# ARISE-Initiative/robosuite

Measured on AMD Instinct MI355X. Metric: env-steps/sec (whole node), Lift/Panda/OSC_POSE @4096 envs/GPU, higher is better.
Workload: dtype f32

## Files before the change

robosuite_amd/csrc/rsim_step.hip:

```cpp
#include <hip/hip_runtime.h>
#include <stdint.h>
#include <type_traits>

#include "../../include/rsim.h"
#include "rsim_internal.h"

#ifndef RSIM_CFG
#define RSIM_CFG 0
#endif
#if RSIM_CFG == 0
#define RSIM_DIMS 32, 16, 16, 24, 16, 16, 64, 192
#define RSIM_SYM(x) x##_cfg0
#define RSIM_DIMS_W 32, 16, 16, 24, 16, 32, 128, 192
#elif RSIM_CFG == 1
#define RSIM_DIMS 32, 16, 32, 24, 16, 32, 64, 192
#define RSIM_SYM(x) x##_cfg1
#define RSIM_DIMS_W 32, 16, 32, 24, 16, 32, 128, 192
#elif RSIM_CFG == 2
#define RSIM_DIMS 64, 16, 16, 32, 32, 32, 64, 320
#define RSIM_SYM(x) x##_cfg2
#define RSIM_DIMS_W 64, 16, 16, 32, 32, 32, 128, 320
#elif RSIM_CFG == 3
#define RSIM_DIMS 64, 32, 48, 64, 32, 32, 128, 640
#define RSIM_SYM(x) x##_cfg3
// ... 2975 lines not shown
    SYNC();
#pragma unroll
    for (int k = 0; k < NA; k++) lt6[k] = Lt[k * NA + (lane & (NA - 1))];
    {
      const float zl = rchol_solve_m<NA>(lr6, lt6, linv6, own6, lane < 6 ? vv[lane] : 0.f);
#pragma unroll
      for (int r = 0; r < 6; r++) z[r] = bcast(zl, r);
      if (!c.uncouple) {
        const float wl = rchol_solve_m<NA>(lr6, lt6, linv6, own6, lane < 3 ? F[lane] : (lane < 6 ? T[lane - 3] : 0.f));
#pragma unroll
        for (int r = 0; r < 6; r++) wrench[r] = bcast(wl, r);
      }
    }
    float tq = 0.f;
    if (lane < n) {
      tq = sm.qfrc_bias[di] + matmp;
#pragma unroll
      for (int r = 0; r < 6; r++) tq = fmaf(comp6(jc, r < 3 ? r + 3 : r - 3), wrench[r] - z[r], tq);
    }
    ctrl_write<ARM>(K, tq);
  }

  struct Row {
    float J[FAST ? NV16 : 1];
    float D, R, aref, fl, mu, fr_own, Dm;
    float fj[CD - 1];
    int row, type, head, kk, dim;
    bool valid, ell;
  };
  __device__ __forceinline__ float row_dot(const Row& rw, float x) const {
    if constexpr (FAST) return dot_rows<NV16>(rw.J, x);
    else return j_row_dot(rw.row * JS, x);
  }
  __device__ __forceinline__ float j_row_dot(int base, float x) const {
    if constexpr (!JG) return lds_row_dot(sm.J + base, x);
    else {
      float a[NV16];
#pragma unroll
      for (int u = 0; u < NV16; u++) a[u] = Jg[base + u];
      float acc = 0.f;
#pragma unroll
      for (int u = 0; u < NV16; u++) acc = fmaf(a[u], bcast(x, u), acc);
      return acc;
    }
  }
  __device__ __forceinline__ double row_res64(const Row& rw, float x, float xl) const {
    return j_row_res64(rw.row * JS, x, xl, rw.aref);
  }
  __device__ __forceinline__ double j_row_res64(int base, float x, float xl, float aref) const {
    if constexpr (!JG) return lds_row_res64(sm.J + base, x, xl, aref);
    else {
      float a[NV16];
#pragma unroll
      for (int u = 0; u < NV16; u++) a[u] = Jg[base + u];
      double acc = -(double)aref;
      float lo = 0.f;
#pragma unroll
      for (int u = 0; u < NV16; u++) { acc = fma((double)a[u], (double)bcast(x, u), acc); lo = fmaf(a[u], bcast(xl, u), lo); }
      return acc + (double)lo;
    }
  }
  __device__ __forceinline__ float lds_row_dot(const float* p, float x) const {
    float acc = 0.f;
    for (int k0 = 0; k0 < m.nv; k0 += 16) {
      float a[16];
#pragma unroll
      for (int u = 0; u < 16; u++) a[u] = p[k0 + u];
#pragma unroll
      for (int u = 0; u < 16; u++) acc = fmaf(a[u], bcast(x, k0 + u), acc);
    }
    return acc;
  }
  __device__ __forceinline__ double lds_row_res64(const float* p, float x, float xl, float aref) const {
    double acc = -(double)aref;
    float lo = 0.f;
    for (int k0 = 0; k0 < m.nv; k0 += 16) {
      float a[16];
#pragma unroll
      for (int u = 0; u < 16; u++) a[u] = p[k0 + u];
#pragma unroll
      for (int u = 0; u < 16; u++) { acc = fma((double)a[u], (double)bcast(x, k0 + u), acc); lo = fmaf(a[u], bcast(xl, k0 + u), lo); }
    }
    return acc + (double)lo;
  }
  __device__ __forceinline__ float mass_dot(const float (&Mr)[FAST ? NV16 : 1], float x) const {
    if constexpr (FAST) return dot_rows<NV16>(Mr, x);
    else {
      float acc;
      if constexpr (MG) {
        float a[NV16];
        const int base = (lane < m.nv ? lane : 0) * NVP;
#pragma unroll
        for (int u = 0; u < NV16; u++) a[u] = Mg[base + u];
        acc = 0.f;
#pragma unroll
        for (int u = 0; u < NV16; u++) acc = fmaf(a[u], bcast(x, u), acc);
      } else acc = lds_row_dot(sm.M + (lane < m.nv ? lane : 0) * NVP, x);
      return lane < m.nv ? acc : 0.f;
    }
  }
  __device__ __forceinline__ void gather(const Row (&rw)[NSLOT], const float (&x)[NSLOT], float (&out)[NSLOT][CD]) const {
    float u[NSLOT];
#pragma unroll
    for (int s = 0; s < NSLOT; s++) u[s] = x[s] * rw[s].fr_own;
#pragma unroll
    for (int s = 0; s < NSLOT; s++)
#pragma unroll
      for (int j = 0; j < CD; j++) {
        const int R = rw[s].head + j;
        float t = __shfl(u[0], R & 63);
#pragma unroll
        for (int s2 = 1; s2 < NSLOT; s2++) { const float t1 = __shfl(u[s2], R & 63); t = (R >> 6) == s2 ? t1 : t; }
        out[s][j] = (rw[s].ell && j < rw[s].dim) ? t : 0.f;
      }
  }
  __device__ __forceinline__ float row_update(const Row& rw, float x, float& force, int& state, const float (&uj)[CD], float& T, float& g) const {
    float cost = 0.f;
    force = 0.f; state = ST_SATISFIED; T = 0.f; g = 0.f;
    if (!rw.valid) return 0.f;
    if (rw.type == C_FRICTION_DOF) {
      if (x <= -rw.R * rw.fl) { state = ST_LINEARNEG; force = rw.fl; cost = rw.fl * (-0.5f * rw.R * rw.fl - x); }
      else if (x >= rw.R * rw.fl) { state = ST_LINEARPOS; force = -rw.fl; cost = rw.fl * (-0.5f * rw.R * rw.fl + x); }
      else { state = ST_QUADRATIC; force = -rw.D * x; cost = 0.5f * rw.D * x * x; }
    } else if (TENDONS && rw.type == C_EQUALITY) {
      state = ST_QUADRATIC; force = -rw.D * x; cost = 0.5f * rw.D * x * x;
    } else if (!rw.ell) {
      if (x < 0) { state = ST_QUADRATIC; force = -rw.D * x; cost = 0.5f * rw.D * x * x; }
    } else {
      float N = uj[0], T2 = 0.f;
#pragma unroll
      for (int j = 1; j < CD; j++) T2 = fmaf(uj[j], uj[j], T2);
      T = sqrtf(T2);
      const float mu = rw.mu;
      if (N >= mu * T || (T <= 0 && N >= 0)) {
      } else if (mu * N + T <= 0 || (T <= 0 && N < 0)) {
        state = ST_QUADRATIC; force = -rw.D * x; cost = 0.5f * rw.D * x * x;
      } else {
        g = N - mu * T;
        float f0 = -rw.Dm * g * mu;
        state = ST_CONE;
        if (rw.kk == 0) { force = f0; cost = 0.5f * rw.Dm * g * g; }
        else force = -f0 / T * (x * rw.fr_own) * rw.fr_own;
      }
    }
    return cost;
  }
  __device__ __forceinline__ void row_ls(const Row& rw, float jar, float jv, const float (&g0)[CD], const float (&gv)[CD], float alpha, float& c, float& c1, float& c2) const {
    c = c1 = c2 = 0.f;
    if (!rw.valid) return;
    float x = fmaf(alpha, jv, jar), v = jv;
    if (rw.type == C_FRICTION_DOF) {
      if (x <= -rw.R * rw.fl) { c = rw.fl * (-0.5f * rw.R * rw.fl - x); c1 = -rw.fl * v; }
      else if (x >= rw.R * rw.fl) { c = rw.fl * (-0.5f * rw.R * rw.fl + x); c1 = rw.fl * v; }
      else { c = 0.5f * rw.D * x * x; c1 = rw.D * x * v; c2 = rw.D * v * v; }
    } else if (TENDONS && rw.type == C_EQUALITY) {
      c = 0.5f * rw.D * x * x; c1 = rw.D * x * v; c2 = rw.D * v * v;
    } else if (!rw.ell) {
      if (x < 0) { c = 0.5f * rw.D * x * x; c1 = rw.D * x * v; c2 = rw.D * v * v; }
    } else {
      const float mu = rw.mu;
      float N = fmaf(alpha, gv[0], g0[0]), T2 = 0.f, UV = 0.f, VV = 0.f;
#pragma unroll
      for (int j = 1; j < CD; j++) { float U = fmaf(alpha, gv[j], g0[j]); T2 = fmaf(U, U, T2); UV = fmaf(U, gv[j], UV); VV = fmaf(gv[j], gv[j], VV); }
      float T = sqrtf(T2);
      if (N >= mu * T || (T <= 0 && N >= 0)) {
      } else if (mu * N + T <= 0 || (T <= 0 && N < 0)) {
        c = 0.5f * rw.D * x * x; c1 = rw.D * x * v; c2 = rw.D * v * v;
      } else if (rw.kk == 0) {
        float g = N - mu * T, iT = 1.0f / T;
        float g1 = gv[0] - mu * UV * iT, g2 = -mu * (VV * iT - UV * UV * iT * iT * iT);
        c = 0.5f * rw.Dm * g * g; c1 = rw.Dm * g * g1; c2 = rw.Dm * (g1 * g1 + g * g2);
      }
    }
  }
  template <int NBT>
  __device__ __forceinline__ void jtf_wide(int nch) {
    if constexpr (NBT <= NT) {
      v4f acc[NBT];
#pragma unroll
      for (int t = 0; t < NBT; t++) acc[t] = v4f{0.f, 0.f, 0.f, 0.f};
      const int q = lane >> 4, col = lane & 15;
      for (int c0 = 0; c0 < nch; c0 += 2) {
        float ja[2][NBT], fb[2];
#pragma unroll
        for (int u = 0; u < 2; u++) {
          const int r = 4 * (c0 + u) + q;
          fb[u] = sm.e_force[r];
#pragma unroll
          for (int t = 0; t < NBT; t++) ja[u][t] = Jrd(r * JS + 16 * t + col);
        }
#pragma unroll
        for (int u = 0; u < 2; u++)
#pragma unroll
          for (int t = 0; t < NBT; t++) acc[t] = __builtin_amdgcn_mfma_f32_16x16x4f32(ja[u][t], fb[u], acc[t], 0, 0, 0);
      }
      if (col == 0) {
#pragma unroll
        for (int t = 0; t < NBT; t++) { float* o = sm.red + 16 * t + 4 * q; o[0] = acc[t][0]; o[1] = acc[t][1]; o[2] = acc[t][2]; o[3] = acc[t][3]; }
      }
    }
  }
  template <int NBT>
  __device__ __forceinline__ void hess_wide(int nch) {
    if constexpr (NBT <= NT) {
      constexpr int NTL = NBT * (NBT + 1) / 2;
      const int q = lane >> 4, col = lane & 15;
      v4f acc[NTL];
      {
        int t = 0;
#pragma unroll
        for (int ti = 0; ti < NBT; ti++)
#pragma unroll
          for (int tj = 0; tj <= ti; tj++, t++)
#pragma unroll
            for (int v = 0; v < 4; v++) acc[t][v] = Mrd((16 * ti + 4 * q + v) * NVP + 16 * tj + col);
      }
      float cf[4];
      int bd;
      {
        const float* o = sm.u.W + 5 * q;
        cf[0] = o[0]; cf[1] = o[1]; cf[2] = o[2]; cf[3] = o[3]; bd = ((const int*)o)[4];
      }
      for (int c = 0; c < nch; c++) {
        const int r = 4 * c + q;
        float cfn[4];
        int bdn;
        {
          const float* o = sm.u.W + 5 * (r + 4 < NEFCAP ? r + 4 : r);
          cfn[0] = o[0]; cfn[1] = o[1]; cfn[2] = o[2]; cfn[3] = o[3]; bdn = ((const int*)o)[4];
        }
        float bj[NBT], aj[NBT];
#pragma unroll
        for (int t = 0; t < NBT; t++) bj[t] = Jrd(r * JS + 16 * t + col);
        if (__ballot((bd >> 16) & 1)) {
          const int head = bd & 255, dm1 = ((bd >> 8) & 7) - 1;
          const int j0 = head * JS + col;
          const int o1 = (dm1 < 1 ? dm1 : 1) * JS, o2 = (dm1 < 2 ? dm1 : 2) * JS, o3 = (dm1 < 3 ? dm1 : 3) * JS;
          float x0[NBT], x1[NBT], x2[NBT], x3[NBT];
#pragma unroll
          for (int t = 0; t < NBT; t++) { x0[t] = Jrd(j0 + 16 * t); x1[t] = Jrd(j0 + o1 + 16 * t); x2[t] = Jrd(j0 + o2 + 16 * t); x3[t] = Jrd(j0 + o3 + 16 * t); }
#pragma unroll
          for (int t = 0; t < NBT; t++) aj[t] = fmaf(cf[3], x3[t], fmaf(cf[2], x2[t], fmaf(cf[1], x1[t], cf[0] * x0[t])));
        } else {
#pragma unroll
          for (int t = 0; t < NBT; t++) aj[t] = cf[0] * bj[t];
        }
        {
          int t = 0;
#pragma unroll
          for (int ti = 0; ti < NBT; ti++)
#pragma unroll
            for (int tj = 0; tj <= ti; tj++, t++) acc[t] = __builtin_amdgcn_mfma_f32_16x16x4f32(aj[ti], bj[tj], acc[t], 0, 0, 0);
        }
#pragma unroll
        for (int k = 0; k < 4; k++) cf[k] = cfn[k];
        bd = bdn;
      }
      {
        int t = 0;
#pragma unroll
        for (int ti = 0; ti < NBT; ti++)
#pragma unroll
          for (int tj = 0; tj <= ti; tj++, t++)
#pragma unroll
            for (int v = 0; v < 4; v++) sm.H[(16 * ti + 4 * q + v) * NVP + 16 * tj + col] = acc[t][v];
      }
    }
  }
  __device__ __forceinline__ float jt_times_force(int nch) {
#pragma unroll
    for (int t = 0; t < (FAST ? NT : 0); t++) {
      v4f acc = {0.f, 0.f, 0.f, 0.f};
      if constexpr (FAST) {
        for (int c0 = 0; c0 < nch; c0 += 4) {
          float ja[4], fb[4];
#pragma unroll
          for (int u = 0; u < 4; u++) { const int r = 4 * (c0 + u) + (lane >> 4); ja[u] = Jrd(r * JS + (lane & 15)); fb[u] = sm.e_force[r]; }
#pragma unroll
          for (int u = 0; u < 4; u++) acc = __builtin_amdgcn_mfma_f32_16x16x4f32(ja[u], fb[u], acc, 0, 0, 0);
        }
      }
      if constexpr (FAST) if ((lane & 15) == 0) { float* o = sm.red + 16 * t + 4 * (lane >> 4); o[0] = acc[0]; o[1] = acc[1]; o[2] = acc[2]; o[3] = acc[3]; }
    }
    if constexpr (!FAST) {
      switch ((m.nv + 15) >> 4) {
        case 1: jtf_wide<1>(nch); break;
        case 2: jtf_wide<2>(nch); break;
        case 3: jtf_wide<3>(nch); break;
        default: jtf_wide<4>(nch); break;
      }
    }
    SYNC();
    float r = FAST ? sm.red[lane & 15] : (lane < NV16 ? sm.red[lane] : 0.f);
    SYNC();
    return r;
  }

  __device__ __forceinline__ void solve_newton() {
    const int nv = m.nv, n = sm.nefc;
    const int nch = (n + 3) >> 2, nvt = (nv + 15) & ~15;
    const float scale = 1.0f / (m.meaninertia * (nv > 1 ? nv : 1));
    const float tolerance = m.tolerance;
#define SLOT_ON(s) (64 * (s) < n || (s) == 0)
    Row rw[NSLOT];
#pragma unroll
    for (int s = 0; s < NSLOT; s++) {
      Row& w_ = rw[s];
      const int row = lane + 64 * s;
      w_.row = row;
      w_.valid = row < n;
      const int r = w_.valid ? row : 0;
      if constexpr (FAST) {
#pragma unroll
        for (int k = 0; k < NV16; k++) w_.J[k] = Jrd(row * JS + k);
      }
      const int desc = w_.valid ? sm.e_desc[r] : 0;
      w_.type = w_.valid ? (desc & 15) : -1;
      const bool tfric = TENDONS && w_.type == C_FRICTION_TENDON;
      if (tfric) w_.type = C_FRICTION_DOF;
      w_.R = sm.e_R[r]; w_.D = 1.0f / w_.R; w_.aref = w_.valid ? sm.e_aref[r] : 0.f; w_.fl = tfric ? FP(FO_tendon_fl, (desc >> 4) & 255) : (w_.type == C_FRICTION_DOF ? cmf(MK_fricFl)->fricFl[(desc >> 4) & 255] : 0.f);
      w_.ell = w_.type == C_CONTACT_ELLIPTIC;
      const int c = w_.ell ? (desc >> 4) & 255 : 0;
      w_.kk = w_.ell ? (desc >> 12) & 15 : 0; w_.head = row - w_.kk; w_.dim = w_.ell ? sm.cdim[c] : 1;
      w_.mu = sm.cmu[c];
#pragma unroll
      for (int j = 0; j < CD - 1; j++) w_.fj[j] = cfri_rd(5 * c + j);
      w_.fr_own = w_.kk == 0 ? w_.mu : cfri_rd(5 * c + w_.kk - 1);
      w_.Dm = (1.0f / sm.e_R[w_.ell ? w_.head : r]) / fmaxf(w_.mu * w_.mu * (1 + w_.mu * w_.mu), 1e-15f);
    }
    const int rr = FAST ? (lane & 15) : lane;
    const bool dofl = lane < NV16;
    float Mr[FAST ? NV16 : 1];
    v4f Macc = {0.f, 0.f, 0.f, 0.f};
    if constexpr (FAST) {
#pragma unroll
      for (int k = 0; k < NV16; k++) Mr[k] = (rr < nv && k < nv) ? sm.M[rr * NVP + k] : 0.f;
#pragma unroll
      for (int v = 0; v < 4; v++) { int i = 4 * (lane >> 4) + v, j = lane & 15; Macc[v] = (i < nv && j < nv) ? sm.M[i * NVP + j] : (i == j ? 1.f : 0.f); }
    }
    SUBMARK(RP_X0);
    const float a_sm = rr < nv ? sm.qacc_smooth[rr] : 0.f, a_ws = rr < nv ? sm.qacc_ws[rr] : 0.f, f_sm = rr < nv ? sm.qfrc_smooth[rr] : 0.f;
    float force[NSLOT], jar[NSLOT], uj[NSLOT][CD], T[NSLOT], g[NSLOT];
    int state[NSLOT];
#pragma unroll
    for (int s = 0; s < NSLOT; s++) { force[s] = 0.f; jar[s] = 0.f; T[s] = 0.f; g[s] = 0.f; state[s] = ST_SATISFIED; }
    auto evaluate = [&](float x) -> float {
#pragma unroll
      for (int s = 0; s < NSLOT; s++) if SLOT_ON(s) jar[s] = row_dot(rw[s], x) - rw[s].aref;
      gather(rw, jar, uj);
      float c = 0.f;
#pragma unroll
      for (int s = 0; s < NSLOT; s++) if SLOT_ON(s) c += row_update(rw[s], jar[s], force[s], state[s], uj[s], T[s], g[s]);
      return c;
    };
    auto weights = [&]() {
#pragma unroll
      for (int s = 0; s < NSLOT; s++) {
        const Row& w_ = rw[s];
        const float dq = state[s] == ST_QUADRATIC ? w_.D : 0.f;
        float hk[CD];
#pragma unroll
        for (int k2 = 0; k2 < CD; k2++) hk[k2] = 0.f;
        if (state[s] == ST_CONE) {
          const float mu = w_.mu, iT = 1.0f / T[s];
          const float uo = jar[s] * w_.fr_own;
          const float grj = w_.kk == 0 ? mu : -mu * uo * w_.fr_own * iT;
#pragma unroll
          for (int k2 = 0; k2 < CD; k2++) {
            if (k2 < w_.dim) {
              const float frk = k2 == 0 ? mu : w_.fj[k2 > 0 ? k2 - 1 : 0];
              const float grk = k2 == 0 ? mu : -mu * uj[s][k2] * frk * iT;
              float h = grj * grk;
              if (w_.kk > 0 && k2 > 0) h += -g[s] * mu * w_.fr_own * frk * ((w_.kk == k2 ? iT : 0.f) - uo * uj[s][k2] * iT * iT * iT);
              hk[k2] = h * w_.Dm;
            }
          }
        }
        if constexpr (FAST) {
          float w[NV16];
#pragma unroll
          for (int k = 0; k < NV16; k++) w[k] = dq * w_.J[k];
          if (state[s] == ST_CONE) {
#pragma unroll
            for (int k2 = 0; k2 < CD; k2++) {
              if (k2 < w_.dim) {
                const int js = (w_.head + k2) * JS;
#pragma unroll
                for (int k = 0; k < NV16; k++) w[k] = fmaf(hk[k2], Jrd(js + k), w[k]);
              }
            }
          }
#pragma unroll
          for (int k = 0; k < NV16; k++) sm.u.W[w_.row * JS + k] = w[k];
        } else {
          if SLOT_ON(s) {
            float* o = sm.u.W + 5 * w_.row;
            const bool cone = state[s] == ST_CONE;
            o[0] = cone ? hk[0] : dq; o[1] = hk[1]; o[2] = hk[2]; o[3] = hk[3];
            ((int*)o)[4] = cone ? (w_.head | (w_.dim << 8) | (1 << 16)) : (w_.row | (1 << 8));
          }
        }
      }
    };
    bool factored = false;
    int fst[NSLOT];
#pragma unroll
    for (int s = 0; s < NSLOT; s++) fst[s] = ST_SATISFIED;
    auto factorize = [&]() {
      if constexpr (!FAST) {
        switch ((nv + 15) >> 4) {
          case 1: hess_wide<1>(nch); break;
          case 2: hess_wide<2>(nch); break;
          case 3: hess_wide<3>(nch); break;
          default: hess_wide<4>(nch); break;
        }
        SYNC();
        SUBMARK_H(RP_X7);
        bchol_inplace<NVP>(sm.H, sm.invdiag, nv, lane);
        factored = true;
#pragma unroll
        for (int s = 0; s < NSLOT; s++) fst[s] = state[s];
        SUBMARK_H(RP_X8);
      }
    };
    float cost_sm = wave_sum(evaluate(a_sm));
    float cost_ws = wave_sum(evaluate(a_ws));
    {
      const float dws = a_ws - a_sm, sv = mass_dot(Mr, dws);
      cost_ws += wave_sum(dofl ? 0.5f * sv * dws : 0.f);
    }
    SUBMARK(RP_X1);
    float a = cost_ws < cost_sm ? a_ws : a_sm;
    int iter = 0;
    bool have_eval = false;
    int pol_exit = 0, pol_pass = 0, pol_sgb = 0;
    float cost_pre = 0.f;
    for (;;) {
      float cost = have_eval ? cost_pre : wave_sum(evaluate(a));
      have_eval = false;
      int state0[NSLOT];
#pragma unroll
      for (int s = 0; s < NSLOT; s++) state0[s] = state[s];
      const float ma = mass_dot(Mr, a);
      const float gauss = wave_sum(dofl ? 0.5f * (ma - f_sm) * (a - a_sm) : 0.f);
      cost += gauss;
#pragma unroll
      for (int s = 0; s < NSLOT; s++) sm.e_force[lane + 64 * s] = force[s];
      SYNC();
      const float jf = jt_times_force(nch);
      float gk = rr < nv ? ma - f_sm - jf : 0.f;
      const float gn = wave_sum(dofl ? gk * gk : 0.f);
      SUBMARK(RP_X2);
      if (iter >= m.iterations || scale * sqrtf(gn) < tolerance) break;
      if (m.newton_ng > 0.f && !__ballot(dofl && rr < nv && fabsf(gk) > m.newton_ng * (fabsf(ma) + fabsf(f_sm) + fabsf(jf)))) break;
      weights();
      SYNC();
      float sk;
      SUBMARK(RP_X3);
      if constexpr (!FAST) {
        factorize();
        sk = bchol_solve<NVP>(sm.H, sm.invdiag, lane < nv ? -gk : 0.f, nv, lane);
        if (lane >= nv) sk = 0.f;
        SUBMARK_H(RP_X9);
      } else {
        v4f acc = Macc;
        for (int c0 = 0; c0 < nch; c0 += 4) {
          float wa[4], jb[4];
#pragma unroll
          for (int u = 0; u < 4; u++) { const int o = (4 * (c0 + u) + (lane >> 4)) * JS + (lane & 15); wa[u] = sm.u.W[o]; jb[u] = Jrd(o); }
#pragma unroll
          for (int u = 0; u < 4; u++) acc = __builtin_amdgcn_mfma_f32_16x16x4f32(wa[u], jb[u], acc, 0, 0, 0);
        }
#pragma unroll
        for (int v = 0; v < 4; v++) sm.H[(4 * (lane >> 4) + v) * NVP + (lane & 15)] = acc[v];
        SYNC();
        float hr[NV16], hinv[NV16], ht[NV16];
        const int rr2 = lane & 15;
#pragma unroll
        for (int k = 0; k < NV16; k++) hr[k] = sm.H[rr2 * NVP + k];
        const int ro = opaque_lane(rr2);
        const float hown = rchol_factor_own<NV16>(hr, hinv, ro);
        rchol_mask_lower<NV16>(hr, ro);
        SYNC();
        if (lane < NV16) {
#pragma unroll
          for (int k = 0; k < NV16; k++) sm.H[lane * NVP + k] = hr[k];
        }
        SYNC();
#pragma unroll
        for (int k = 0; k < NV16; k++) ht[k] = sm.H[k * NVP + rr2];
        sk = rchol_solve_m<NV16>(hr, ht, hinv, hown, rr2 < nv ? -gk : 0.f);
        if (rr2 >= nv) sk = 0.f;
      }
      SUBMARK(RP_X4);
      float jv[NSLOT];
#pragma unroll
      for (int s = 0; s < NSLOT; s++) jv[s] = SLOT_ON(s) ? row_dot(rw[s], sk) : 0.f;
      const float mvv = mass_dot(Mr, sk);
      const float q1 = wave_sum(dofl ? sk * (ma - f_sm) : 0.f), q2 = wave_sum(dofl ? 0.5f * sk * mvv : 0.f), sn = sqrtf(wave_sum(dofl ? sk * sk : 0.f));
      if (sn < 1e-15f) break;
      float g0[NSLOT][CD], gvv[NSLOT][CD];
      gather(rw, jar, g0);
      gather(rw, jv, gvv);
      const float gtol = tolerance * 0.01f * sn / scale;
      float p0, d0, h0, p, dp, hp, lo = 0.f, hi = -1.f, alpha;
      auto line = [&](float al, float& c, float& c1, float& c2) {
        c = c1 = c2 = 0.f;
#pragma unroll
        for (int s = 0; s < NSLOT; s++) if SLOT_ON(s) { float t, t1, t2; row_ls(rw[s], jar[s], jv[s], g0[s], gvv[s], al, t, t1, t2); c += t; c1 += t1; c2 += t2; }
      };
      {
        float c, c1, c2;
        line(0.f, c, c1, c2);
        p0 = gauss + wave_sum(c); d0 = q1 + wave_sum(c1); h0 = 2 * q2 + wave_sum(c2);
      }
      SUBMARK(RP_X5);
      if (d0 >= 0 || h0 <= 0) break;
      alpha = -d0 / h0;
      const float dtol = fmaxf(gtol, 1e-6f * fabsf(d0));
      const float atol = ((FAST || m.newton_wide) && m.newton_ls > 0.f && m.newton_ns > 0.f)
                             ? m.newton_ls * wave_min_f((dofl && rr < nv && sk != 0.f) ? (m.newton_ns * fabsf(a) + m.newton_na) / fabsf(sk) : 3.0e38f) : 0.f;
      bool at_alpha = false;
      for (int ls = 0; ls < m.ls_iterations; ls++) {
        pf.count(RP_N_LS, 1);
        float c, c1, c2;
        line(alpha, c, c1, c2);
        p = gauss + alpha * q1 + alpha * alpha * q2 + wave_sum(c);
        dp = q1 + 2 * alpha * q2 + wave_sum(c1);
        hp = 2 * q2 + wave_sum(c2);
        at_alpha = true;
        if (fabsf(dp) < dtol) break;
        if (dp < 0) lo = alpha; else hi = alpha;
        float next = hp > 0 ? alpha - dp / hp : -1.f;
        if (hi < 0) { if (next <= lo) next = 2 * alpha + 1e-12f; }
        else if (next <= lo || next >= hi) next = 0.5f * (lo + hi);
        if (fabsf(next - alpha) <= fmaxf(1e-6f * fabsf(alpha), atol)) break;
        alpha = next;
        at_alpha = false;
      }
      if (!at_alpha) {
        float c, c1, c2;
        line(alpha, c, c1, c2);
        p = gauss + alpha * q1 + alpha * alpha * q2 + wave_sum(c);
      }
      SUBMARK(RP_X6);
      if (!(p < p0)) break;
      const float a_new = fmaf(alpha, sk, a);
      const bool settled = (FAST || m.newton_wide == 1) && m.newton_ns > 0.f && !__ballot(dofl && rr < nv && fabsf(alpha * sk) > m.newton_ns * fabsf(a_new) + m.newton_na);
      a = a_new;
      iter++;
      if (scale * (p0 - p) < tolerance || settled) {
        evaluate(a);
        break;
      }
      if (m.newton_exact) {
        cost_pre = wave_sum(evaluate(a));
        have_eval = true;
        bool moved = false;
#pragma unroll
        for (int s = 0; s < NSLOT; s++) if SLOT_ON(s) moved |= rw[s].valid && (state[s] != state0[s] || state0[s] == ST_CONE);
        if (!__ballot(moved)) break;
      }
    }
    if constexpr (!FAST && POLISH) {
      const int R = m.newton_refine;
      if (R > 0 && n > 0) {
        bool need_factor = !factored;
        float a_lo = 0.f, a_keep = a, alo_keep = 0.f, force_keep[NSLOT], dk = 0.f;
        int state_keep[NSLOT];
        double err_keep = 1.0e300;
#pragma unroll
        for (int s = 0; s < NSLOT; s++) { force_keep[s] = force[s]; state_keep[s] = state[s]; }
        auto dfadd = [](float& hi, float& lo, float d) {
          const float sm_ = __fadd_rn(hi, d), bb = __fsub_rn(sm_, hi), se = __fadd_rn(__fsub_rn(hi, __fsub_rn(sm_, bb)), __fsub_rn(d, bb));
          const float l2 = __fadd_rn(lo, se);
          hi = __fadd_rn(sm_, l2);
          lo = __fsub_rn(l2, __fsub_rn(hi, sm_));
        };
        int flat = 0;
        bool use_ls = m.newton_polish_gate < 0.f;
        double gn_prev = 1.0e300;
        for (int it = 0;;) {
          double jr[NSLOT], u64[NSLOT], c64 = 0.0;
#pragma unroll
          for (int s = 0; s < NSLOT; s++) { jr[s] = SLOT_ON(s) ? row_res64(rw[s], a, a_lo) : 0.0; u64[s] = jr[s] * (double)rw[s].fr_own; }
#pragma unroll
          for (int s = 0; s < NSLOT; s++) {
            const Row& w_ = rw[s];
            double uj64[CD];
#pragma unroll
            for (int j = 0; j < CD; j++) {
              const int Rr = w_.head + j;
              double t = __shfl(u64[0], Rr & 63);
#pragma unroll
              for (int s2 = 1; s2 < NSLOT; s2++) { const double t1 = __shfl(u64[s2], Rr & 63); t = (Rr >> 6) == s2 ? t1 : t; }
              uj64[j] = (w_.ell && j < w_.dim) ? t : 0.0;
            }
            double f = 0.0, Tn = 0.0, gg = 0.0;
            int st = ST_SATISFIED;
            if (w_.valid && SLOT_ON(s)) {
              const double x = jr[s], D = (double)w_.D;
              if (w_.type == C_FRICTION_DOF) {
                const double fl = (double)w_.fl, lim = (double)w_.R * fl;
                if (x <= -lim) { st = ST_LINEARNEG; f = fl; c64 += fl * (-0.5 * lim - x); }
                else if (x >= lim) { st = ST_LINEARPOS; f = -fl; c64 += fl * (-0.5 * lim + x); }
                else { st = ST_QUADRATIC; f = -D * x; c64 += 0.5 * D * x * x; }
              } else if (TENDONS && w_.type == C_EQUALITY) {
                st = ST_QUADRATIC; f = -D * x; c64 += 0.5 * D * x * x;
              } else if (!w_.ell) {
                if (x < 0) { st = ST_QUADRATIC; f = -D * x; c64 += 0.5 * D * x * x; }
              } else {
                const double N = uj64[0], mu = (double)w_.mu;
                double T2 = 0.0;
#pragma unroll
                for (int j = 1; j < CD; j++) T2 = fma(uj64[j], uj64[j], T2);
                Tn = sqrt(T2);
                if (N >= mu * Tn || (Tn <= 0 && N >= 0)) {
                } else if (mu * N + Tn <= 0 || (Tn <= 0 && N < 0)) {
                  st = ST_QUADRATIC; f = -D * x; c64 += 0.5 * D * x * x;
                } else {
                  gg = N - mu * Tn;
                  const double f0 = -(double)w_.Dm * gg * mu;
                  st = ST_CONE;
                  if (w_.kk == 0) { f = f0; c64 += 0.5 * (double)w_.Dm * gg * gg; }
                  else f = -f0 / Tn * u64[s] * (double)w_.fr_own;
                }
              }
            }
            state[s] = st; jar[s] = (float)jr[s]; T[s] = (float)Tn; g[s] = (float)gg;
#pragma unroll
            for (int j = 0; j < CD; j++) uj[s][j] = (float)uj64[j];
            force[s] = (float)f;
            if SLOT_ON(s) {
              sm.u.W[w_.row] = force[s];
              sm.u.W[NEFCAP + w_.row] = (float)(f - (double)force[s]);
            }
          }
          SYNC();
          double gk = 0.0, ma64 = 0.0;
          if (lane < nv) {
            double ma = 0.0, jf = 0.0;
            for (int j = 0; j < nv; j++) ma = fma((double)Mrd(lane * NVP + j), (double)bcast(a, j) + (double)bcast(a_lo, j), ma);
            for (int r = 0; r < n; r++) jf = fma((double)Jrd(r * JS + lane), (double)sm.u.W[r] + (double)sm.u.W[NEFCAP + r], jf);
            gk = ma - (double)f_sm - jf; ma64 = ma;
            c64 += 0.5 * (ma - (double)f_sm) * ((double)a + (double)a_lo - (double)a_sm);
          }
          const double err = wave_sum_f64(c64);
          if (!(err <= err_keep + 1e-12 * fabs(err_keep))) {
            a = a_keep; a_lo = alo_keep;
            if (!use_ls && NSLOT <= RSIM_LS_MAXSLOT) {
              use_ls = true; err_keep = 1.0e300;
              SYNC();
              continue;
            }
#pragma unroll
            for (int s = 0; s < NSLOT; s++) { force[s] = force_keep[s]; state[s] = state_keep[s]; }
            pol_exit = 6; pol_pass = it;
            break;
          }
          const double gain = err_keep - err;
          bool flipped = false;
#pragma unroll
          for (int s = 0; s < NSLOT; s++) if SLOT_ON(s) flipped |= rw[s].valid && state[s] != state_keep[s];
          flipped = __ballot(flipped) != 0;
          a_keep = a; alo_keep = a_lo; err_keep = err;
#pragma unroll
          for (int s = 0; s < NSLOT; s++) { force_keep[s] = force[s]; state_keep[s] = state[s]; }
          const double gn = wave_sum_f64(lane < nv ? gk * gk : 0.0);
          const double sg = (double)scale * sqrt(gn), tol64 = (double)tolerance * (double)m.newton_polish_tol;
          { const int bk = sg > 0.0 ? (int)(-log10(sg)) : 15; pol_sgb = bk < 0 ? 0 : (bk > 15 ? 15 : bk); pol_pass = it; }
          if (sg < tol64) { pol_exit = 1; break; }
          if (it > 0 && !flipped && (double)scale * gain < tol64) { if (++flat >= 3) { pol_exit = 2; break; } } else flat = 0;
          if (it >= R) { pol_exit = 3; break; }
          if (it > 0 && gn > 0.0625 * gn_prev) use_ls = true;
          gn_prev = gn;
          it++;
          bool other = false;
#pragma unroll
          for (int s = 0; s < NSLOT; s++) if SLOT_ON(s) other |= rw[s].valid && (state[s] != fst[s] || (it >= 2 && state[s] == ST_CONE));
          SYNC();
          if (__ballot(other) || need_factor) {
            need_factor = false;
            weights();
            SYNC();
            factorize();
          }
          dk = bchol_solve<NVP>(sm.H, sm.invdiag, lane < nv ? -(float)gk : 0.f, nv, lane);
          if (lane >= nv) dk = 0.f;
          double alpha = 1.0;
          if (use_ls && NSLOT <= RSIM_LS_MAXSLOT) {
            double jv[NSLOT], v64[NSLOT], g0[NSLOT][CD], gv[NSLOT][CD];
#pragma unroll
            for (int s = 0; s < NSLOT; s++) { jv[s] = SLOT_ON(s) ? row_res64(rw[s], dk, 0.f) + (double)rw[s].aref : 0.0; v64[s] = jv[s] * (double)rw[s].fr_own; }
#pragma unroll
            for (int s = 0; s < NSLOT; s++)
#pragma unroll
              for (int j = 0; j < CD; j++) {
                const int Rr = rw[s].head + j;
                double tu = __shfl(u64[0], Rr & 63), tv = __shfl(v64[0], Rr & 63);
#pragma unroll
                for (int s2 = 1; s2 < NSLOT; s2++) { const double t1 = __shfl(u64[s2], Rr & 63), t2 = __shfl(v64[s2], Rr & 63); if ((Rr >> 6) == s2) { tu = t1; tv = t2; } }
                const bool on = rw[s].ell && j < rw[s].dim;
                g0[s][j] = on ? tu : 0.0; gv[s][j] = on ? tv : 0.0;
              }
            const double mvv = (double)mass_dot(Mr, dk);
            const double q1 = wave_sum_f64(lane < nv ? (double)dk * (ma64 - (double)f_sm) : 0.0), q2 = wave_sum_f64(lane < nv ? 0.5 * (double)dk * mvv : 0.0);
            auto line64 = [&](double al, double& d1, double& d2) {
              d1 = d2 = 0.0;
#pragma unroll
              for (int s = 0; s < NSLOT; s++) {
                const Row& w_ = rw[s];
                if (!(w_.valid && SLOT_ON(s))) continue;
                const double x = fma(al, jv[s], jr[s]), v = jv[s], D = (double)w_.D;
                if (w_.type == C_FRICTION_DOF) {
                  const double fl = (double)w_.fl, lim = (double)w_.R * fl;
                  if (x <= -lim) d1 -= fl * v; else if (x >= lim) d1 += fl * v; else { d1 += D * x * v; d2 += D * v * v; }
                } else if (TENDONS && w_.type == C_EQUALITY) { d1 += D * x * v; d2 += D * v * v; }
                else if (!w_.ell) { if (x < 0) { d1 += D * x * v; d2 += D * v * v; } }
                else {
                  const double mu = (double)w_.mu, N = fma(al, gv[s][0], g0[s][0]);
                  double T2 = 0.0, UV = 0.0, VV = 0.0;
#pragma unroll
                  for (int j = 1; j < CD; j++) { const double U = fma(al, gv[s][j], g0[s][j]); T2 = fma(U, U, T2); UV = fma(U, gv[s][j], UV); VV = fma(gv[s][j], gv[s][j], VV); }
                  const double Tn = sqrt(T2);
                  if (N >= mu * Tn || (Tn <= 0 && N >= 0)) {
                  } else if (mu * N + Tn <= 0 || (Tn <= 0 && N < 0)) { d1 += D * x * v; d2 += D * v * v; }
                  else if (w_.kk == 0) {
                    const double g_ = N - mu * Tn, iT = 1.0 / Tn, g1 = gv[s][0] - mu * UV * iT, g2 = -mu * (VV * iT - UV * UV * iT * iT * iT);
                    d1 += (double)w_.Dm * g_ * g1; d2 += (double)w_.Dm * (g1 * g1 + g_ * g2);
                  }
                }
              }
            };
            double c1, c2;
            line64(0.0, c1, c2);
            const double d0 = q1 + wave_sum_f64(c1), h0 = 2.0 * q2 + wave_sum_f64(c2);
            if (!(d0 < 0.0) || !(h0 > 0.0)) {
              pol_exit = 5; break;
            }
            alpha = -d0 / h0;
            double lo = 0.0, hi = -1.0;
            bool conv = false;
            for (int ls = 0; ls < 24; ls++) {
              line64(alpha, c1, c2);
              const double dp = q1 + 2.0 * alpha * q2 + wave_sum_f64(c1), hp = 2.0 * q2 + wave_sum_f64(c2);
              if (fabs(dp) < 1e-9 * fabs(d0)) { conv = true; break; }
              if (dp < 0) lo = alpha; else hi = alpha;
              double next = hp > 0 ? alpha - dp / hp : -1.0;
              if (hi < 0) { if (next <= lo) next = 2.0 * alpha + 1e-12; }
              else if (next <= lo || next >= hi) next = 0.5 * (lo + hi);
              if (fabs(next - alpha) <= 1e-12 * fabs(alpha)) { conv = true; break; }
              alpha = next;
            }
            if (!conv && lo > 0.0) alpha = lo;
            if (conv && hi > 0.0 && hi - lo <= 1e-6 * hi) alpha = hi;
          }
          dfadd(a, a_lo, (float)(alpha * (double)dk));
          SYNC();
        }
      }
    }
#pragma unroll
    for (int s = 0; s < NSLOT; s++) sm.e_force[lane + 64 * s] = force[s];
    SYNC();
    const float fc = jt_times_force(nch);
    if (lane < nv) { sm.qfrc_constraint[lane] = fc; sm.qacc[lane] = a; }
    if (lane == 0) { sm.niter = iter; sm.polish = 10000 * pol_pass + 100000 * pol_sgb + 10000000 * pol_exit; }
    pf.count(RP_N_NEWTON, iter);
    SYNC();
#undef SLOT_ON
  }


  __device__ __forceinline__ Q4 mat2quat_xyzw(const float* R) const {
    const float m00 = R[0], m01 = R[1], m02 = R[2], m10 = R[3], m11 = R[4], m12 = R[5], m20 = R[6], m21 = R[7], m22 = R[8];
    float qw, qx, qy, qz;
    const float tr = m00 + m11 + m22;
    if (tr > 0.f) { const float sq = sqrtf(tr + 1.f) * 2.f; qw = 0.25f * sq; qx = (m21 - m12) / sq; qy = (m02 - m20) / sq; qz = (m10 - m01) / sq; }
    else if (m00 > m11 && m00 > m22) { const float sq = sqrtf(1.f + m00 - m11 - m22) * 2.f; qw = (m21 - m12) / sq; qx = 0.25f * sq; qy = (m01 + m10) / sq; qz = (m02 + m20) / sq; }
    else if (m11 > m22) { const float sq = sqrtf(1.f + m11 - m00 - m22) * 2.f; qw = (m02 - m20) / sq; qx = (m01 + m10) / sq; qy = 0.25f * sq; qz = (m12 + m21) / sq; }
    else { const float sq = sqrtf(1.f + m22 - m00 - m11) * 2.f; qw = (m10 - m01) / sq; qx = (m02 + m20) / sq; qy = (m12 + m21) / sq; qz = 0.25f * sq; }
    if (qw < 0.f) { qw = -qw; qx = -qx; qy = -qy; qz = -qz; }
    Q4 q = {qw, qx, qy, qz};
    return q;
  }
  __device__ __forceinline__ void peg_orientation(int peg, int hole, float& tt, float& dd, float& cs) const {
    const M3 Rp = q2m(ldq(sm.xquat + 4 * peg)), Rh = q2m(ldq(sm.xquat + 4 * hole));
    const V3 pp = ld3(sm.xpos + 3 * peg), hp = ld3(sm.xpos + 3 * hole);
    V3 v = col(Rp, 2);
    v = v * (1.0f / norm(v));
    const V3 center = hp + col(Rh, 0) * 0.1f;
    const float vn = norm(v);
    tt = dot(center - pp, v) / (vn * vn);
    dd = norm(cross(v, pp - center)) / vn;
    const V3 hn = col(Rh, 2);
    cs = fabsf(dot(hn, v) / norm(hn) / vn);
  }
  __device__ __forceinline__ void obs_reward(float* obs, float* __restrict__ reward, int* __restrict__ success, bool reset_obs) {
    const DTask& t = m.task;
    gci prog = (gci)t.obs_prog;
    float peg_t = 0.f, peg_d = 0.f, peg_c = 0.f;
    if (t.task == 3) peg_orientation(t.object_body, t.object2_body, peg_t, peg_d, peg_c);
    float* prev = sm.u.b.poly;
    if (t.task == 4) {
      if (lane < 7 * t.nobj) prev[lane] = obs[seli(t.pos_slot, lane / 7) + lane % 7];
      SYNC();
    }
    for (int i = lane; i < t.nobs; i += 64) {
      const int kind = prog[3 * i], a = prog[3 * i + 1], b2 = prog[3 * i + 2];
      float v = 0.f;
      if (kind == RSIM_OBS_QPOS) v = sm.qpos[a];
      else if (kind == RSIM_OBS_COS) { float sn, cs; sincos_f(sm.qpos[a], sn, cs); v = cs; }
      else if (kind == RSIM_OBS_SIN) { float sn, cs; sincos_f(sm.qpos[a], sn, cs); v = sn; }
      else if (kind == RSIM_OBS_QVEL) v = sm.qvel[a];
      else if (kind == RSIM_OBS_QACC) v = sm.qacc[a];
      else if (kind == RSIM_OBS_SITE_POS) v = sm.spos[3 * a + b2];
      else if (kind == RSIM_OBS_BODY_POS) v = sm.xpos[3 * (a < 0 ? seli(t.obj_body, task_obj) : a) + b2];
      else if (kind == RSIM_OBS_TASK_OBJECT) v = (float)task_obj;
      else if (kind == RSIM_OBS_BODY_MINUS_SITE) v = sm.xpos[3 * a + (b2 & 3)] - sm.spos[3 * (b2 >> 2) + (b2 & 3)];
      else if (kind == RSIM_OBS_BODY_MINUS_BODY) v = sm.xpos[3 * a + (b2 & 3)] - sm.xpos[3 * (b2 >> 2) + (b2 & 3)];
      else if (kind == RSIM_OBS_REL_POS || kind == RSIM_OBS_REL_QUAT) {
        if (!reset_obs) {
          const float* o = prev + 7 * (a < 0 ? task_obj : a);
          const Q4 qo = {o[6], o[3], o[4], o[5]};
          const M3 Re = q2m(ldq(sm.xquat + 4 * t.eef_body)), Ro = q2m(qnorm(qo));
          if (kind == RSIM_OBS_REL_POS) {
            const V3 r = mtv(Re, v3(o[0], o[1], o[2]) - ld3(sm.spos + 3 * t.grip_site));
            v = b2 == 0 ? r.x : (b2 == 1 ? r.y : r.z);
          } else {
            const M3 Rr = mtm(Re, Ro);
            const Q4 q = mat2quat_xyzw(Rr.m);
            v = b2 == 0 ? q.x : (b2 == 1 ? q.y : (b2 == 2 ? q.z : q.w));
          }
        }
      }
      else if (kind == RSIM_OBS_PEG_COS) v = peg_c;
      else if (kind == RSIM_OBS_PEG_T) v = peg_t;
      else if (kind == RSIM_OBS_PEG_D) v = peg_d;
      else if (kind == RSIM_OBS_BODY_QUAT) v = sm.xquat[4 * (a < 0 ? seli(t.obj_body, task_obj) : a) + (b2 == 3 ? 0 : b2 + 1)];
      else if (kind == RSIM_OBS_SITE_QUAT) { const Q4 q = mat2quat_xyzw(sm.smat + 9 * a); v = b2 == 0 ? q.x : (b2 == 1 ? q.y : (b2 == 2 ? q.z : q.w)); }
      obs[i] = v;
    }
    if (t.task == 4) {
      const int i = lane < t.nobj ? lane : 0;
      const V3 op = ld3(sm.xpos + 3 * seli(t.obj_body, i)), grip = ld3(sm.spos + 3 * t.grip_site);
      const float dist = norm(grip - op);
      float bxl = t.bin2_pos[0], byl = t.bin2_pos[1];
      if (i == 0 || i == 2) bxl -= t.bin_size[0] * 0.5f;
      if (i < 2) byl -= t.bin_size[1] * 0.5f;
      const bool inside = bxl < op.x && op.x < bxl + t.bin_size[0] * 0.5f && byl < op.y && op.y < byl + t.bin_size[1] * 0.5f && t.bin2_pos[2] < op.z && op.z < t.bin2_pos[2] + 0.1f;
      const bool in_bin = lane < t.nobj && inside && (1.f - tanhf(10.f * dist)) < 0.6f;
      const bool activeo = lane < t.nobj && !in_bin;
      const u64 act_mask = __ballot(activeo), in_mask = __ballot(in_bin);
      u64 ageoms = 0;
#pragma unroll
      for (int k = 0; k < 4; k++) if ((act_mask >> k) & 1ull) ageoms |= t.obj_geoms[k];
      bool lc = false, rc = false;
      if (lane < sm.ncon) {
        const u64 b1 = 1ull << (sm.cg1[lane] & 255), b2 = 1ull << (sm.cg2[lane] & 255);
        const bool o1 = (ageoms & b1) != 0, o2 = (ageoms & b2) != 0;
        lc = (o1 && (t.left_pad & b2)) || (o2 && (t.left_pad & b1));
        rc = (o1 && (t.right_pad & b2)) || (o2 && (t.right_pad & b1));
      }
      const bool grasp = __ballot(lc) != 0 && __ballot(rc) != 0;
      const float BIG = 3.0e38f;
      const float dmin = wave_min_f(activeo ? dist : BIG);
      const float zd = fmaxf(t.bin2_pos[2] + 0.25f - op.z, 0.f), zmin = wave_min_f(activeo ? zd : BIG);
      const float r_reach = act_mask ? (1.f - tanhf(10.f * dmin)) * 0.1f : 0.f;
      const float r_grasp = grasp ? 0.35f : 0.f;
      const float r_lift = (act_mask && grasp) ? 0.35f + (1.f - tanhf(15.f * zmin)) * 0.15f : 0.f;
      const float tx = sel(t.bin_target, 2 * i), ty = sel(t.bin_target, 2 * i + 1);
      const bool above = fabsf(op.x - tx) < t.bin_size[0] * 0.25f && fabsf(op.y - ty) < t.bin_size[1] * 0.25f;
      const float dxy = sqrtf((tx - op.x) * (tx - op.x) + (ty - op.y) * (ty - op.y));
      const float hov = (above ? 0.5f : r_lift) + (1.f - tanhf(10.f * dxy)) * 0.2f;
      const float r_hover = act_mask ? wave_max(activeo ? hov : -BIG) : 0.f;
      if (lane == 0) {
        const int nin = __popcll(in_mask);
        float r = (float)nin;
        if (t.reward_shaping) r += fmaxf(fmaxf(r_reach, r_grasp), fmaxf(r_lift, r_hover));
        if (reward) { *reward = t.single_mode ? r * t.reward_scale : r * t.reward_scale / 4.0f; *success = (t.single_mode ? nin > 0 : nin == t.nobj) ? 1 : 0; }
      }
    } else if (t.task == 3) {
      if (lane == 0) {
        const bool succ = peg_d < 0.06f && peg_t >= -0.12f && peg_t <= 0.14f && peg_c > 0.95f;
        float r = succ ? 1.f : 0.f;
        if (t.reward_shaping) {
          const float dist = norm(ld3(sm.xpos + 3 * t.object_body) - ld3(sm.xpos + 3 * t.object2_body));
          r += (1.f - tanhf(dist)) + (1.f - tanhf(peg_d)) + (1.f - tanhf(fabsf(peg_t))) + peg_c;
        } else r *= 5.f;
        if (reward) { *reward = r * t.reward_scale / 5.0f; *success = succ ? 1 : 0; }
      }
    } else if (t.task >= 1) {
      bool lc = false, rc = false, oo = false;
      if (lane < sm.ncon) {
        const unsigned long long b1 = 1ull << (sm.cg1[lane] & 255), b2 = 1ull << (sm.cg2[lane] & 255);
        const bool obj1 = (t.object_geoms & b1) != 0, obj2 = (t.object_geoms & b2) != 0;
        lc = (obj1 && (t.left_pad & b2)) || (obj2 && (t.left_pad & b1));
        rc = (obj1 && (t.right_pad & b2)) || (obj2 && (t.right_pad & b1));
        oo = (obj1 && (t.object2_geoms & b2)) || (obj2 && (t.object2_geoms & b1));
      }
      const bool grasp = __ballot(lc) != 0 && __ballot(rc) != 0;
      const bool touching = __ballot(oo) != 0;
      if (lane == 0 && t.task == 2) {
        const V3 cA = ld3(sm.xpos + 3 * t.object_body), cB = ld3(sm.xpos + 3 * t.object2_body), grip = ld3(sm.spos + 3 * t.grip_site);
        float r_reach = (1.f - tanhf(10.f * norm(cA - grip))) * 0.25f;
        if (grasp) r_reach += 0.25f;
        const bool lifted = cA.z > t.table_height + t.lift_margin;
        float r_lift = lifted ? 1.f : 0.f;
        if (lifted) { const float dx = cA.x - cB.x, dy = cA.y - cB.y; r_lift += 0.5f * (1.f - tanhf(sqrtf(dx * dx + dy * dy))); }
        const float r_stack = (!grasp && r_lift > 0.f && touching) ? 2.f : 0.f;
        const float r = t.reward_shaping ? fmaxf(r_reach, fmaxf(r_lift, r_stack)) : r_stack;
        if (reward) { *reward = r * t.reward_scale / 2.0f; *success = r_stack > 0.f ? 1 : 0; }
      }
      if (lane == 0 && t.task == 1) {
        const V3 cube = ld3(sm.xpos + 3 * t.object_body), grip = ld3(sm.spos + 3 * t.grip_site);
        const bool succ = cube.z > t.table_height + t.lift_margin;
        float r = 0.f;
        if (succ) r = 2.25f;
        else if (t.reward_shaping) { r = 1.f - tanhf(10.f * norm(cube - grip)); if (grasp) r += 0.25f; }
        if (reward) { *reward = r * t.reward_scale / 2.25f; *success = succ ? 1 : 0; }
      }
    }
  }

  __device__ __forceinline__ void fwd_constraint() {
    if (sm.nefc == 0) {
      if (lane < m.nv) { sm.qacc[lane] = sm.qacc_smooth[lane]; sm.qfrc_constraint[lane] = 0.f; }
      if (lane == 0) sm.niter = 0;
      SYNC();
      return;
    }
    solve_newton();
  }
};

struct Handover { int sub0; float time; bool fresh_ctrl, handed; int ndiverged, need_con, need_efc; float cstate; unsigned t_launch;
                  bool restarted; };

template <int NB, int NJ, int NV, int NG, int NS, int NCON, int NEFC, int NPAIR, bool DBG, int FUSED = 0, bool PLAIN = false>
__device__ __forceinline__ bool step_body(const DModel& m, const DBatch& b, const float* __restrict__ actions, int n_sub, int flags, int slot, Handover* ho = nullptr) {
  typedef Smem<NB, NJ, NV, NG, NS, NCON, NEFC, NPAIR> SM;
  const int lane = FUSED ? opaque_lane((int)threadIdx.x) : (int)threadIdx.x;
  const bool reentry = FUSED == 1 && (flags & RF_RESET_ONLY);
  const int tpass = (!DBG && b.tier_cur && !reentry) ? (FUSED == 2 ? 2 : FUSED == 1 ? 0 : b.tier_pass) : -1;
  const bool resume = FUSED == 2 && ho->sub0 > 0;
  if ((tpass <= 0 || FUSED) && slot >= (b.nenv ? b.nenv : b.B)) return false;
  const int env = uni((tpass > 0 && !FUSED) ? b.wlist[slot] : (b.order ? b.order[slot] : slot) + b.env0);
  if (!reentry && (flags & RF_RESET_ONLY) && !b.needs_reset[env]) return false;
  if (!FUSED && tpass == 0 && b.tier_cur[env] != 0) return false;
  const unsigned t_launch = resume ? ho->t_launch : ((b.cost && !reentry) ? (unsigned)uni((int)(clock64() >> 6)) : 0u);
  const float* fp = m.ft + (size_t)env * m.fstride;
  typedef Sim<SM, PLAIN> SimT;
  SimT sim(m, fp, lane, PLAIN ? nullptr : b.prof, b.cm, b.cm_stride ? (const char*)b.cm_env + (size_t)env * b.cm_stride : (const char*)b.cm);
  if constexpr (!PLAIN) {
    sim.pf.acc = b.prof_env == -1 || b.prof_env == env;
    if (b.prof) sim.pf.pairs = b.prof + RP_COUNT + 8 * (size_t)b.B;
  }
  sim.pf.start();
  if (!PLAIN && b.prof && lane == 0 && !resume) {
    unsigned long long* wl = b.prof + RP_COUNT + 8 * (size_t)env;
    wl[0] = (unsigned)__builtin_amdgcn_s_getreg((31 << 11) | 4);
    wl[1] = (unsigned)__builtin_amdgcn_s_getreg((31 << 11) | 20);
    wl[2] = wall_clock64();
  }
  if (!resume) {
    for (int i = lane; i < m.nq; i += 64) sm.qpos[i] = b.qpos[(size_t)env * m.nq + i];
    for (int i = lane; i < m.nv; i += 64) { sm.qvel[i] = b.qvel[(size_t)env * m.nv + i]; sm.qacc_ws[i] = b.qacc_ws[(size_t)env * m.nv + i]; }
    if (lane >= m.nv && lane < NV) { sm.qvel[lane] = 0.f; sm.qacc_ws[lane] = 0.f; sm.qacc[lane] = 0.f; }
    for (int i = lane; i < m.nu; i += 64) sm.ctrl[i] = b.ctrl[(size_t)env * m.nu + i];
  }
  const int cs = m.ctrl.cs_size, csl = cs < RSIM_CS_LDS ? cs : RSIM_CS_LDS;
  sim.cst = (gwf)(b.cstate + (size_t)env * cs);
  if (b.bpl) sim.bpl = (int __attribute__((address_space(1)))*)(b.bpl + (size_t)env * 320);
  if (b.mprc) { sim.mprc = (gwf)(b.mprc + (size_t)env * SimT::MPRC * m.npair); sim.mpr_portal = b.mprc_portal != 0; }
  if constexpr (SimT::JG) sim.Jg = (gwf)(b.jg + (size_t)env * b.jg_stride);
  if constexpr (SimT::MG) sim.Mg = sim.Jg + SM::NEFC_ * SM::JS_;
  if (lane < csl) sm.cstate[lane] = resume ? ho->cstate : sim.cst[lane];
  gcf qfa = nullptr, xfa = nullptr;
  u64 xmask = 0;
  if (!PLAIN && (DBG || (flags & RF_APPLIED))) {
    if (b.qfrc_applied) qfa = (gcf)(b.qfrc_applied + (size_t)env * m.nv);
    if (b.xfrc_applied) {
      xfa = (gcf)(b.xfrc_applied + (size_t)env * m.nbody * 6);
      bool nz = false;
      if (lane < m.nbody) for (int k = 0; k < 6; k++) nz |= xfa[6 * lane + k] != 0.f;
      xmask = __ballot(nz);
    }
  }
  if (lane == 0) { sm.ncon = 0; sm.nefc = 0; sm.niter = 0; sm.polish = 0; }
  sim.load_opt();
  sim.init_lds();
  const float* act = actions ? actions + (size_t)env * m.ctrl.action_dim : nullptr;
  float time = __builtin_bit_cast(float, uni(__builtin_bit_cast(int, b.time[env])));
  bool fresh_ctrl = false;
  int ndiverged = 0;
  if (resume) { time = ho->time; fresh_ctrl = ho->fresh_ctrl; ndiverged = ho->ndiverged; sim.need_con = ho->need_con; sim.need_efc = ho->need_efc; }
  if (!resume && (flags & RF_CTRL) && b.needs_reset[env]) {
    V3 xp0; Q4 xq0;
    if (lane < csl) sm.cstate[lane] = 0.f;
    for (int i = RSIM_CS_LDS + lane; i < cs; i += 64) sim.cst[i] = 0.f;
    SYNC();
    sim.cst_sync();
    sim.kinematics(xp0, xq0);
    sim.geom_site_frames();
    sim.ctrl_reset();
    fresh_ctrl = true;
  }
  sim.pf.mark(RP_LOAD);
  int sub = resume ? ho->sub0 : 0;
  bool over = false;
  const int force_sub = (FUSED == 1 && b.tier_pass >= 100) ? b.tier_pass - 100 : -1;
  for (; sub < n_sub; sub++) {
    V3 xp; Q4 xq;
    sim.phase();
    sim.kinematics(xp, xq);
    sim.phase();
    sim.geom_site_frames();
    sim.pf.mark(RP_KIN);
    sim.phase();
    sim.com_pos(xp, xq);
    sim.pf.mark(RP_COM);
    sim.phase();
    sim.crb();
    sim.pf.mark(RP_CRB);
    sim.phase();
    sim.collision(n_sub - sub);
    sim.pf.mark(RP_NARROW);
    if (FUSED == 1 && tpass == 0 && (uni(sim.ovf) || sub == force_sub)) { over = true; break; }
    sim.phase();
    sim.make_constraint();
    sim.pf.mark(RP_MAKEC);
    if (FUSED == 1 && tpass == 0 && uni(sim.ovf)) { over = true; break; }
    sim.phase();
    sim.velocity(xp, xq);
    sim.pf.mark(RP_VEL);
    if (flags & RF_CTRL) {
      sim.phase();
      if ((flags & RF_SETGOAL) && sub == 0 && act) {
        const float* act0 = act;
        asm volatile("" : "+s"(act0));
        sim.ctrl_set_goal(act0);
      }
      sim.ctrl_run();
      sim.pf.mark(RP_CTRL);
    }
    if (flags & RF_ACTSOLVE) {
      sim.phase();
      if constexpr (PLAIN) sim.actuation_acceleration(); else sim.actuation_acceleration(qfa, xfa, xmask);
      sim.pf.mark(RP_ACT);
      sim.phase();
      sim.fwd_constraint();
      sim.pf.mark(RP_SOLVE);
      sim.pf.count(RP_N_CON, sm.ncon);
      sim.pf.count(RP_N_EFC, sm.nefc);
      if constexpr (DBG) {
        if ((flags & RF_DEBUG) && b.sensordata && m.nsensor > 0 && sub == n_sub - 1) { sim.phase(); sim.sensor_acc(xp, xq, b.sensordata + (size_t)env * m.nsensordata, xfa, xmask); }
      }
    }
    if (flags & RF_INTEGRATE) {
      sim.phase();
      sim.euler();
      sim.pf.mark(RP_EULER);
      time += sim.opt_h;
      bool bad = false;
#ifdef RSIM_GUARD_LANE
      const int gl = sim.lane;
#else
      const int gl = lane;
// ... 408 lines not shown
```

Before: 1.371 million.

## Reuse warm-start evaluation and final J^T f; build Hessian weights on the fly

```diff
diff --git a/robosuite_amd/csrc/rsim_step.hip b/robosuite_amd/csrc/rsim_step.hip
--- a/robosuite_amd/csrc/rsim_step.hip
+++ b/robosuite_amd/csrc/rsim_step.hip
@@ -3301,6 +3301,13 @@
     const float scale = 1.0f / (m.meaninertia * (nv > 1 ? nv : 1));
     const float tolerance = m.tolerance;
 #define SLOT_ON(s) (64 * (s) < n || (s) == 0)
+#ifdef RSIM_SOLVER_REPEAT_PASSES
+    constexpr bool REUSE_START = false, REUSE_JF = false, STORED_W = true;
+#elif defined(RSIM_FAST_STORED_W)
+    constexpr bool REUSE_START = true, REUSE_JF = true, STORED_W = true;
+#else
+    constexpr bool REUSE_START = true, REUSE_JF = true, STORED_W = false;
+#endif
     Row rw[NSLOT];
 #pragma unroll
     for (int s = 0; s < NSLOT; s++) {
@@ -3375,7 +3382,7 @@
             }
           }
         }
-        if constexpr (FAST) {
+        if constexpr (FAST && STORED_W) {
           float w[NV16];
 #pragma unroll
           for (int k = 0; k < NV16; k++) w[k] = dq * w_.J[k];
@@ -3392,7 +3399,7 @@
 #pragma unroll
           for (int k = 0; k < NV16; k++) sm.u.W[w_.row * JS + k] = w[k];
         } else {
-          if SLOT_ON(s) {
+          if (FAST || SLOT_ON(s)) {
             float* o = sm.u.W + 5 * w_.row;
             const bool cone = state[s] == ST_CONE;
             o[0] = cone ? hk[0] : dq; o[1] = hk[1]; o[2] = hk[2]; o[3] = hk[3];
@@ -3423,7 +3430,8 @@
       }
     };
     float cost_sm = wave_sum(evaluate(a_sm));
-    float cost_ws = wave_sum(evaluate(a_ws));
+    const float rows_ws = wave_sum(evaluate(a_ws));
+    float cost_ws = rows_ws;
     {
       const float dws = a_ws - a_sm, sv = mass_dot(Mr, dws);
       cost_ws += wave_sum(dofl ? 0.5f * sv * dws : 0.f);
@@ -3431,9 +3439,11 @@
     SUBMARK(RP_X1);
     float a = cost_ws < cost_sm ? a_ws : a_sm;
     int iter = 0;
-    bool have_eval = false;
     int pol_exit = 0, pol_pass = 0, pol_sgb = 0;
-    float cost_pre = 0.f;
+    bool have_eval = REUSE_START && cost_ws < cost_sm;
+    float cost_pre = rows_ws;
+    bool jf_final = false;
+    float jf_keep = 0.f;
     for (;;) {
       float cost = have_eval ? cost_pre : wave_sum(evaluate(a));
       have_eval = false;
@@ -3450,8 +3460,8 @@
       float gk = rr < nv ? ma - f_sm - jf : 0.f;
       const float gn = wave_sum(dofl ? gk * gk : 0.f);
       SUBMARK(RP_X2);
-      if (iter >= m.iterations || scale * sqrtf(gn) < tolerance) break;
-      if (m.newton_ng > 0.f && !__ballot(dofl && rr < nv && fabsf(gk) > m.newton_ng * (fabsf(ma) + fabsf(f_sm) + fabsf(jf)))) break;
+      if (iter >= m.iterations || scale * sqrtf(gn) < tolerance) { jf_final = REUSE_JF; jf_keep = jf; break; }
+      if (m.newton_ng > 0.f && !__ballot(dofl && rr < nv && fabsf(gk) > m.newton_ng * (fabsf(ma) + fabsf(f_sm) + fabsf(jf)))) { jf_final = REUSE_JF; jf_keep = jf; break; }
       weights();
       SYNC();
       float sk;
@@ -3465,8 +3475,36 @@
         v4f acc = Macc;
         for (int c0 = 0; c0 < nch; c0 += 4) {
           float wa[4], jb[4];
-#pragma unroll
-          for (int u = 0; u < 4; u++) { const int o = (4 * (c0 + u) + (lane >> 4)) * JS + (lane & 15); wa[u] = sm.u.W[o]; jb[u] = Jrd(o); }
+          if constexpr (STORED_W) {
+#pragma unroll
+            for (int u = 0; u < 4; u++) { const int o = (4 * (c0 + u) + (lane >> 4)) * JS + (lane & 15); wa[u] = sm.u.W[o]; jb[u] = Jrd(o); }
+          } else {
+            float c0f[4];
+            int bd[4];
+#pragma unroll
+            for (int u = 0; u < 4; u++) {
+              const int r = 4 * (c0 + u) + (lane >> 4);
+              const float* o = sm.u.W + 5 * r;
+              c0f[u] = o[0]; bd[u] = ((const int*)o)[4]; jb[u] = Jrd(r * JS + (lane & 15));
+            }
+#pragma unroll
+            for (int u = 0; u < 4; u++) {
+              wa[u] = __fmul_rn(c0f[u], jb[u]);
+              const bool cone = (bd[u] >> 16) & 1;
+              if (__ballot(cone)) {
+                const float* o = sm.u.W + 5 * (4 * (c0 + u) + (lane >> 4));
+                const int dim = (bd[u] >> 8) & 7, j0 = (bd[u] & 255) * JS + (lane & 15);
+                const float h1 = o[1], h2 = o[2], h3 = o[3];
+                const float x0 = Jrd(j0), x1 = Jrd(j0 + (dim > 1 ? 1 : 0) * JS), x2 = Jrd(j0 + (dim > 2 ? 2 : dim - 1) * JS), x3 = Jrd(j0 + (dim > 3 ? 3 : dim - 1) * JS);
+                float w = __fmul_rn(0.f, jb[u]);
+                w = fmaf(c0f[u], x0, w);
+                w = dim > 1 ? fmaf(h1, x1, w) : w;
+                w = dim > 2 ? fmaf(h2, x2, w) : w;
+                w = dim > 3 ? fmaf(h3, x3, w) : w;
+                wa[u] = cone ? w : wa[u];
+              }
+            }
+          }
 #pragma unroll
           for (int u = 0; u < 4; u++) acc = __builtin_amdgcn_mfma_f32_16x16x4f32(wa[u], jb[u], acc, 0, 0, 0);
         }
@@ -3565,6 +3603,7 @@
       const int R = m.newton_refine;
       if (R > 0 && n > 0) {
         bool need_factor = !factored;
+        jf_final = false;
         float a_lo = 0.f, a_keep = a, alo_keep = 0.f, force_keep[NSLOT], dk = 0.f;
         int state_keep[NSLOT];
         double err_keep = 1.0e300;
@@ -3762,7 +3801,7 @@
 #pragma unroll
     for (int s = 0; s < NSLOT; s++) sm.e_force[lane + 64 * s] = force[s];
     SYNC();
-    const float fc = jt_times_force(nch);
+    const float fc = jf_final ? jf_keep : jt_times_force(nch);
     if (lane < nv) { sm.qfrc_constraint[lane] = fc; sm.qacc[lane] = a; }
     if (lane == 0) { sm.niter = iter; sm.polish = 10000 * pol_pass + 100000 * pol_sgb + 10000000 * pol_exit; }
     pf.count(RP_N_NEWTON, iter);
```

After: 1.387 million (median of 4 runs). +1.2%, better.
